# microsoft/ANCE

Measured on NVIDIA H100. Metric: ANN-refresh throughput: passages encoded/sec + queries top-200/sec, 8.8M x 768, higher is better.
Workload: dtype fp16

## Files before the change

### ance_b200/csrc/capi.cu

```cuda
#include <atomic>
#include <mutex>
#include <string.h>
#include <vector>

#include "common.h"
#include "gemm_store.cuh"

namespace ance {

static thread_local char g_err[1024] = "";
std::atomic<int64_t> g_launches{0};

void set_error(const char* fmt, ...) {
  va_list ap;
  va_start(ap, fmt);
  vsnprintf(g_err, sizeof(g_err), fmt, ap);
  va_end(ap);
}

void count_launch(int n) { g_launches.fetch_add(n, std::memory_order_relaxed); }

static bool g_prof_on = false;
static std::mutex g_prof_mu;
static std::vector<cudaEvent_t> g_ev_pool;
struct Span { cudaEvent_t a, b; };
static std::vector<Span> g_spans[kNumCls];
static cudaEvent_t g_open[kNumCls];
static double g_ms[kNumCls];
static int64_t g_cnt[kNumCls];

static cudaEvent_t get_event() {
  if (!g_ev_pool.empty()) { cudaEvent_t e = g_ev_pool.back(); g_ev_pool.pop_back(); return e; }
  cudaEvent_t e; cudaEventCreate(&e); return e;
}
void prof_begin(int cls, cudaStream_t st) {
  if (!g_prof_on) return;
  std::lock_guard<std::mutex> lk(g_prof_mu);
  g_open[cls] = get_event();
  cudaEventRecord(g_open[cls], st);
}
void prof_end(int cls, cudaStream_t st) {
  if (!g_prof_on) return;
  std::lock_guard<std::mutex> lk(g_prof_mu);
  cudaEvent_t b = get_event();
  cudaEventRecord(b, st);
  g_spans[cls].push_back({g_open[cls], b});
}

}

extern "C" const char* ance_version(void) { return "ance_b200 0.1 (sm_90a)"; }
extern "C" const char* ance_last_error(void) { return ance::g_err; }
extern "C" int64_t ance_launch_count(void) { return ance::g_launches.load(); }

extern "C" int ance_profile_enable(int on) {
  std::lock_guard<std::mutex> lk(ance::g_prof_mu);
  ance::g_prof_on = on != 0;
  return ANCE_OK;
}

extern "C" int ance_profile_read(double* ms_by_class, int64_t* launches_by_class, int n, int reset) {
  ANCE_REQUIRE(ms_by_class && launches_by_class && n > 0 && n <= ance::kNumCls, "ance_profile_read: bad arguments");
  ANCE_CUDA(cudaDeviceSynchronize());
  std::lock_guard<std::mutex> lk(ance::g_prof_mu);
  for (int c = 0; c < ance::kNumCls; ++c) {
    for (auto& s : ance::g_spans[c]) {
      float ms = 0.f;
      if (cudaEventElapsedTime(&ms, s.a, s.b) == cudaSuccess) { ance::g_ms[c] += ms; ance::g_cnt[c] += 1; }
      ance::g_ev_pool.push_back(s.a);
      ance::g_ev_pool.push_back(s.b);
    }
    ance::g_spans[c].clear();
  }
  for (int c = 0; c < n; ++c) { ms_by_class[c] = ance::g_ms[c]; launches_by_class[c] = ance::g_cnt[c]; }
  if (reset) for (int c = 0; c < ance::kNumCls; ++c) { ance::g_ms[c] = 0; ance::g_cnt[c] = 0; }
  return ANCE_OK;
}

namespace {

template <int BN, int STAGES, int CG, uint32_t FMT>
int run_dbg(const void* A, const void* B, int M, int N, int K, const float* bias, const void* R, int act, void* C,
            float* C32, cudaStream_t st) {
  constexpr int EW = 4;
  using Ep = gemm::EpStore<BN, EW>;
  CUtensorMap tmA, tmB;
  if (!tc05_host::make_tmap_2d_16b(&tmA, A, M, K, K, gemm::BM) ||
      !tc05_host::make_tmap_2d_16b(&tmB, B, N, K, K, BN / CG)) {
    ance::set_error("cuTensorMapEncodeTiled failed (M=%d N=%d K=%d)", M, N, K);
    return ANCE_ERR_CUDA;
  }
  gemm::WorkShape ws = gemm::make_shape(M, N, K, BN, CG, 0);
  typename Ep::Params p;
  memset(&p, 0, sizeof(p));
  if (C && !gemm::make_store_tmap(&p.tmC, C, M, N, N)) {
    ance::set_error("cuTensorMapEncodeTiled failed for the output (M=%d N=%d)", M, N);
    return ANCE_ERR_CUDA;
  }
  if (C && R && !gemm::make_store_tmap(&p.tmR, const_cast<void*>(R), M, N, N)) {
    ance::set_error("cuTensorMapEncodeTiled failed for the residual (M=%d N=%d)", M, N);
    return ANCE_ERR_CUDA;
  }
  p.C = reinterpret_cast<uint16_t*>(C);
  p.C32 = C32;
  p.bias = bias;
  p.R = reinterpret_cast<const uint16_t*>(R);
  p.ldc = N;
  p.ldc32 = N;
  p.ldr = N;
  p.act = act;
  ANCE_CUDA((gemm::launch<Ep, BN, STAGES, CG, EW, FMT>(tmA, tmB, ws, p, 0, st)));
  ance::count_launch(1);
  return ANCE_OK;
}

template <uint32_t FMT>
int dispatch_dbg(int variant, const void* A, const void* B, int M, int N, int K, const float* bias, const void* R,
                 int act, void* C, float* C32, cudaStream_t st) {
  switch (variant) {
    case 0: return run_dbg<128, 4, 1, FMT>(A, B, M, N, K, bias, R, act, C, C32, st);
    case 1: return run_dbg<128, 3, 1, FMT>(A, B, M, N, K, bias, R, act, C, C32, st);
    case 2: return run_dbg<128, 4, 2, FMT>(A, B, M, N, K, bias, R, act, C, C32, st);
    case 3: return run_dbg<64, 6, 2, FMT>(A, B, M, N, K, bias, R, act, C, C32, st);
    case 4: return run_dbg<64, 6, 1, FMT>(A, B, M, N, K, bias, R, act, C, C32, st);
    default: ance::set_error("ance_dbg_gemm: unknown variant %d", variant); return ANCE_ERR_INVALID;
  }
}

}

extern "C" int ance_dbg_gemm(const void* A_dev, const void* B_dev, int M, int N, int K, int fmt, int variant,
                             const float* bias_dev, const void* residual_bf16_dev, int act, void* C_bf16_dev,
                             float* C_f32_dev, void* stream) {
  ANCE_REQUIRE(A_dev && B_dev && M > 0 && N > 0 && K > 0, "ance_dbg_gemm: null operand or empty shape");
  ANCE_REQUIRE(K % 8 == 0 && N % 8 == 0, "ance_dbg_gemm: K and N must be multiples of 8 (16-byte rows)");
  cudaStream_t st = reinterpret_cast<cudaStream_t>(stream);
  if (fmt == ANCE_FMT_BF16)
    return dispatch_dbg<tc05::kFmtBF16>(variant, A_dev, B_dev, M, N, K, bias_dev, residual_bf16_dev, act, C_bf16_dev,
                                        C_f32_dev, st);
  if (fmt == ANCE_FMT_FP16)
    return dispatch_dbg<tc05::kFmtF16>(variant, A_dev, B_dev, M, N, K, bias_dev, residual_bf16_dev, act, C_bf16_dev,
                                       C_f32_dev, st);
  ance::set_error("ance_dbg_gemm: unknown operand format %d", fmt);
  return ANCE_ERR_INVALID;
}
```

### ance_b200/csrc/encoder.cu

```cuda
#include <math.h>
#include <stdlib.h>
#include <string.h>

#include <map>
#include <vector>

#include "attention.cuh"
#include "common.h"
#include "gemm_store.cuh"

namespace {

constexpr float kLog2e = 1.4426950408889634f;

struct EmbedParams {
  const int32_t* ids;
  const int32_t* lens;
  const uint8_t* mask;
  int B, L, H;
  int roberta;
  int pad_id, vocab, max_pos;
  const float* word;
  const float* pos;
  const float* type;
  const float* gamma;
  const float* beta;
  float eps;
  uint16_t* X;
  float* kbias;
  int* err_flag;
  const int32_t* seq_row0;
};

template <int NV, uint32_t FMT>
__global__ void __launch_bounds__(256) embed_ln_kernel(const EmbedParams p) {
  using A16 = act16::Act<FMT>;
  __shared__ int s_pos[512];
  __shared__ int s_warp_cnt[8];
  const int b = blockIdx.x;
  const int warp = threadIdx.x >> 5, lane = threadIdx.x & 31;
  const int32_t* ids = p.ids + static_cast<size_t>(b) * p.L;
  for (int base = 0, carry = 0; base < p.L; base += 256) {
    const int t = base + threadIdx.x;
    const int flag = (t < p.L && ids[t] != p.pad_id) ? 1 : 0;
    const unsigned bal = __ballot_sync(0xffffffffu, flag);
    if (lane == 0) s_warp_cnt[warp] = __popc(bal);
    __syncthreads();
    int pre = carry;
    for (int w2 = 0; w2 < warp; ++w2) pre += s_warp_cnt[w2];
    const int incl = pre + __popc(bal & ((2u << lane) - 1u));
    if (t < p.L) s_pos[t] = p.roberta ? (flag ? incl + p.pad_id : p.pad_id) : t;
    int tot = 0;
    for (int w2 = 0; w2 < 8; ++w2) tot += s_warp_cnt[w2];
    carry += tot;
    __syncthreads();
  }
  const int len = p.lens ? p.lens[b] : 0;
  const bool varlen = p.seq_row0 != nullptr;
  const size_t row0 = varlen ? static_cast<size_t>(p.seq_row0[b]) : static_cast<size_t>(b) * p.L;
  const int t_end = varlen ? min(len, p.L) : p.L;
  for (int t = warp; t < t_end; t += 8) {
    const size_t tok = row0 + t;
    int id = ids[t];
    int ps = s_pos[t];
    if (id < 0 || id >= p.vocab || ps >= p.max_pos) {
      if (lane == 0) atomicOr(p.err_flag, 1);
      id = min(max(id, 0), p.vocab - 1);
      ps = min(ps, p.max_pos - 1);
    }
    const float4* wr = reinterpret_cast<const float4*>(p.word + static_cast<size_t>(id) * p.H);
    const float4* pr = reinterpret_cast<const float4*>(p.pos + static_cast<size_t>(ps) * p.H);
    const float4* tr = reinterpret_cast<const float4*>(p.type);
    float x[NV * 8];
    float sum = 0.f;
#pragma unroll
    for (int v = 0; v < NV; ++v) {
#pragma unroll
      for (int hf = 0; hf < 2; ++hf) {
        const int c4 = (v * 32 + lane) * 2 + hf;
        const float4 a = __ldg(wr + c4), c = __ldg(pr + c4), d = __ldg(tr + c4);
        x[v * 8 + hf * 4 + 0] = (a.x + c.x) + d.x;
        x[v * 8 + hf * 4 + 1] = (a.y + c.y) + d.y;
        x[v * 8 + hf * 4 + 2] = (a.z + c.z) + d.z;
        x[v * 8 + hf * 4 + 3] = (a.w + c.w) + d.w;
      }
#pragma unroll
      for (int i = 0; i < 8; ++i) sum += x[v * 8 + i];
    }
#pragma unroll
    for (int s = 16; s > 0; s >>= 1) sum += __shfl_xor_sync(0xffffffffu, sum, s);
    const float mean = sum / p.H;
    float var = 0.f;
#pragma unroll
    for (int i = 0; i < NV * 8; ++i) {
      const float dlt = x[i] - mean;
      var = fmaf(dlt, dlt, var);
    }
#pragma unroll
    for (int s = 16; s > 0; s >>= 1) var += __shfl_xor_sync(0xffffffffu, var, s);
    const float rstd = rsqrtf(var / p.H + p.eps);
    uint4* out = reinterpret_cast<uint4*>(p.X + tok * p.H);
#pragma unroll
    for (int v = 0; v < NV; ++v) {
      const int col = (v * 32 + lane) * 8;
      const float4 g0 = __ldg(reinterpret_cast<const float4*>(p.gamma + col)), g1 = __ldg(reinterpret_cast<const float4*>(p.gamma + col + 4));
      const float4 b0 = __ldg(reinterpret_cast<const float4*>(p.beta + col)), b1 = __ldg(reinterpret_cast<const float4*>(p.beta + col + 4));
      const float g[8] = {g0.x, g0.y, g0.z, g0.w, g1.x, g1.y, g1.z, g1.w};
      const float bb[8] = {b0.x, b0.y, b0.z, b0.w, b1.x, b1.y, b1.z, b1.w};
      uint32_t h2[4];
#pragma unroll
      for (int q = 0; q < 4; ++q)
        h2[q] = A16::pack2((x[v * 8 + q * 2] - mean) * rstd * g[q * 2] + bb[q * 2],
                           (x[v * 8 + q * 2 + 1] - mean) * rstd * g[q * 2 + 1] + bb[q * 2 + 1]);
      out[v * 32 + lane] = make_uint4(h2[0], h2[1], h2[2], h2[3]);
    }
    if (lane == 0 && !varlen) {
      const bool keep = p.mask ? (p.mask[tok] != 0) : (t < len);
      p.kbias[tok] = keep ? 0.f : -10000.0f * kLog2e;
    }
  }
}

template <int NV, bool kInF32, uint32_t FMT>
__global__ void __launch_bounds__(256) ln_rows_kernel(const void* __restrict__ in, size_t in_ld, int n_rows, int H,
                                                      const float* __restrict__ gamma, const float* __restrict__ beta,
                                                      float eps, uint16_t* __restrict__ out16,
                                                      float* __restrict__ out32) {
  using A16 = act16::Act<FMT>;
  const int lane = threadIdx.x & 31;
  const int row = blockIdx.x * 8 + (threadIdx.x >> 5);
  if (row >= n_rows) return;
  float x[NV * 8];
  float sum = 0.f;
#pragma unroll
  for (int v = 0; v < NV; ++v) {
    const int col = (v * 32 + lane) * 8;
    if (kInF32) {
      const float* r = reinterpret_cast<const float*>(in) + static_cast<size_t>(row) * in_ld + col;
      const float4 a = __ldg(reinterpret_cast<const float4*>(r)), b = __ldg(reinterpret_cast<const float4*>(r + 4));
      x[v * 8 + 0] = a.x; x[v * 8 + 1] = a.y; x[v * 8 + 2] = a.z; x[v * 8 + 3] = a.w;
      x[v * 8 + 4] = b.x; x[v * 8 + 5] = b.y; x[v * 8 + 6] = b.z; x[v * 8 + 7] = b.w;
    } else {
      const uint16_t* r = reinterpret_cast<const uint16_t*>(in) + static_cast<size_t>(row) * in_ld + col;
      const uint4 a = __ldg(reinterpret_cast<const uint4*>(r));
      const uint32_t ah[4] = {a.x, a.y, a.z, a.w};
#pragma unroll
      for (int q = 0; q < 4; ++q) {
        const float2 f = A16::unpack2(ah[q]);
        x[v * 8 + q * 2] = f.x;
        x[v * 8 + q * 2 + 1] = f.y;
      }
    }
#pragma unroll
    for (int i = 0; i < 8; ++i) sum += x[v * 8 + i];
  }
#pragma unroll
  for (int s = 16; s > 0; s >>= 1) sum += __shfl_xor_sync(0xffffffffu, sum, s);
  const float mean = sum / H;
  float var = 0.f;
#pragma unroll
  for (int i = 0; i < NV * 8; ++i) {
    const float d = x[i] - mean;
// ... 110 lines not shown
  const int lane = threadIdx.x & 31;
  const int row0 = (blockIdx.x * 8 + (threadIdx.x >> 5)) * kB;
  if (row0 >= n_rows) return;
  uint4 raw[kB][NV];
  float sum[kB], var[kB], mean[kB], rstd[kB];
#pragma unroll
  for (int b = 0; b < kB; ++b) {
    const int row = min(row0 + b, n_rows - 1);
    const uint4* src = reinterpret_cast<const uint4*>(in + static_cast<size_t>(row) * in_ld);
#pragma unroll
    for (int v = 0; v < NV; ++v) raw[b][v] = __ldg(src + v * 32 + lane);
  }
#pragma unroll
  for (int b = 0; b < kB; ++b) {
    sum[b] = 0.f;
#pragma unroll
    for (int v = 0; v < NV; ++v) {
      const uint32_t w[4] = {raw[b][v].x, raw[b][v].y, raw[b][v].z, raw[b][v].w};
#pragma unroll
      for (int q = 0; q < 4; ++q) {
        const float2 f = A16::unpack2(w[q]);
        sum[b] += f.x;
        sum[b] += f.y;
      }
    }
  }
#pragma unroll
  for (int s = 16; s > 0; s >>= 1) {
#pragma unroll
    for (int b = 0; b < kB; ++b) sum[b] += __shfl_xor_sync(0xffffffffu, sum[b], s);
  }
#pragma unroll
  for (int b = 0; b < kB; ++b) {
    mean[b] = sum[b] / H;
    var[b] = 0.f;
#pragma unroll
    for (int v = 0; v < NV; ++v) {
      const uint32_t w[4] = {raw[b][v].x, raw[b][v].y, raw[b][v].z, raw[b][v].w};
#pragma unroll
      for (int q = 0; q < 4; ++q) {
        const float2 f = A16::unpack2(w[q]);
        const float d0 = f.x - mean[b], d1 = f.y - mean[b];
        var[b] = fmaf(d0, d0, var[b]);
        var[b] = fmaf(d1, d1, var[b]);
      }
    }
  }
#pragma unroll
  for (int s = 16; s > 0; s >>= 1) {
#pragma unroll
    for (int b = 0; b < kB; ++b) var[b] += __shfl_xor_sync(0xffffffffu, var[b], s);
  }
#pragma unroll
  for (int b = 0; b < kB; ++b) rstd[b] = rsqrtf(var[b] / H + eps);
#pragma unroll
  for (int v = 0; v < NV; ++v) {
    const int col = (v * 32 + lane) * 8;
    const float4 g0 = __ldg(reinterpret_cast<const float4*>(gamma + col)), g1 = __ldg(reinterpret_cast<const float4*>(gamma + col + 4));
    const float4 b0 = __ldg(reinterpret_cast<const float4*>(beta + col)), b1 = __ldg(reinterpret_cast<const float4*>(beta + col + 4));
    const float g[8] = {g0.x, g0.y, g0.z, g0.w, g1.x, g1.y, g1.z, g1.w};
    const float bb[8] = {b0.x, b0.y, b0.z, b0.w, b1.x, b1.y, b1.z, b1.w};
#pragma unroll
    for (int b = 0; b < kB; ++b) {
      const uint32_t w[4] = {raw[b][v].x, raw[b][v].y, raw[b][v].z, raw[b][v].w};
      uint32_t o[4];
#pragma unroll
      for (int q = 0; q < 4; ++q) {
        const float2 f = A16::unpack2(w[q]);
        o[q] = A16::pack2((f.x - mean[b]) * rstd[b] * g[q * 2] + bb[q * 2], (f.y - mean[b]) * rstd[b] * g[q * 2 + 1] + bb[q * 2 + 1]);
      }
      if (row0 + b < n_rows) *reinterpret_cast<uint4*>(out16 + static_cast<size_t>(row0 + b) * H + col) = make_uint4(o[0], o[1], o[2], o[3]);
    }
  }
}

__global__ void gather_rows16_by_index_kernel(const uint16_t* __restrict__ src, const int32_t* __restrict__ idx, int n, int H,
                                              uint16_t* __restrict__ dst) {
  const int r = blockIdx.x;
  if (r >= n) return;
  const uint4* s = reinterpret_cast<const uint4*>(src + static_cast<size_t>(idx[r]) * H);
  uint4* o = reinterpret_cast<uint4*>(dst + static_cast<size_t>(r) * H);
  for (int i = threadIdx.x; i < H / 8; i += blockDim.x) o[i] = __ldg(s + i);
}

template <uint32_t FMT>
__global__ void act16_to_f32_kernel(const uint16_t* __restrict__ in, float* __restrict__ out, size_t n) {
  const size_t i = static_cast<size_t>(blockIdx.x) * blockDim.x + threadIdx.x;
  if (i < n) out[i] = act16::Act<FMT>::to_float(in[i]);
}

__global__ void check_finite_kernel(const float* __restrict__ x, size_t n, int* __restrict__ err_flag) {
  bool bad = false;
  for (size_t i = static_cast<size_t>(blockIdx.x) * blockDim.x + threadIdx.x; i < n; i += static_cast<size_t>(gridDim.x) * blockDim.x)
    bad |= !(fabsf(x[i]) <= 3.0e38f);
  if (__any_sync(0xffffffffu, bad) && (threadIdx.x & 31) == 0) atomicOr(err_flag, 2);
}

}

struct LayerDev {
  uint16_t *wqkv, *wo, *w1, *w2;
  float *bqkv, *bo, *b1, *b2, *ln1g, *ln1b, *ln2g, *ln2b;
};

struct ance_encoder {
  ance_encoder_config cfg{};
  int max_tokens = 0;
  uint32_t fmt = tc05::kFmtF16;
  int device = 0;
  float *word = nullptr, *pos = nullptr, *type = nullptr;
  float *eg = nullptr, *eb = nullptr;
  std::vector<LayerDev> layers;
  uint16_t* head_w = nullptr;
  float *head_b = nullptr, *head_g = nullptr, *head_bt = nullptr;
  uint16_t *X = nullptr, *QKV = nullptr, *CTX = nullptr, *T = nullptr, *X1 = nullptr, *FF = nullptr;
  float* kbias = nullptr;
  uint16_t *cls_ctx = nullptr, *cls_x = nullptr;
  int32_t* seq_row0 = nullptr;
  uint8_t *row_lo = nullptr, *row_hi = nullptr;
  float* head_tmp = nullptr;
  int* err_flag = nullptr;
  uint16_t* dbg = nullptr;
  int dbg_tokens = 0;
  int prune_last_layer = 1;
  int varlen_align = 1;
  std::vector<void*> allocs;
};

namespace {

template <class T>
T* dev_alloc(ance_encoder* e, size_t n) {
  void* p = nullptr;
  if (cudaMalloc(&p, n * sizeof(T)) != cudaSuccess) return nullptr;
  e->allocs.push_back(p);
  return reinterpret_cast<T*>(p);
}

float* upload_f32(ance_encoder* e, const float* h, size_t n) {
  float* d = dev_alloc<float>(e, n);
  if (d) cudaMemcpy(d, h, n * 4, cudaMemcpyHostToDevice);
  return d;
}

uint16_t* upload_16(ance_encoder* e, const float* h, size_t n) {
  std::vector<uint16_t> tmp(n);
  if (e->fmt == tc05::kFmtBF16) for (size_t i = 0; i < n; ++i) tmp[i] = act16::Act<tc05::kFmtBF16>::from_float_host(h[i]);
  else for (size_t i = 0; i < n; ++i) tmp[i] = act16::Act<tc05::kFmtF16>::from_float_host(h[i]);
  uint16_t* d = dev_alloc<uint16_t>(e, n);
  if (d) cudaMemcpy(d, tmp.data(), n * 2, cudaMemcpyHostToDevice);
  return d;
}

template <uint32_t FMT>
int linear(const uint16_t* A, size_t lda, int M, const uint16_t* W, int N, int K, const float* bias,
           const uint16_t* R, int act, uint16_t* C, float* C32, cudaStream_t st, int cls = ance::kClsGemm,
           size_t ldr = 0) {
  constexpr int BN = 128, CG = 1, EW = 4, STAGES = 4;
  using Ep = gemm::EpStore<BN, EW, FMT>;
  CUtensorMap tmA, tmB;
  if (!tc05_host::make_tmap_2d_16b(&tmA, A, M, K, lda, gemm::BM) || !tc05_host::make_tmap_2d_16b(&tmB, W, N, K, K, BN / CG)) {
    ance::set_error("encoder: cuTensorMapEncodeTiled failed (M=%d N=%d K=%d)", M, N, K);
    return ANCE_ERR_CUDA;
  }
  gemm::WorkShape ws = gemm::make_shape(M, N, K, BN, CG, 0);
  typename Ep::Params p;
  memset(&p, 0, sizeof(p));
  if (C && !gemm::make_store_tmap(&p.tmC, C, M, N, N)) {
    ance::set_error("encoder: cuTensorMapEncodeTiled failed for the output (M=%d N=%d)", M, N);
    return ANCE_ERR_CUDA;
  }
  if (ldr == 0) ldr = N;
  if (C && R && !gemm::make_store_tmap(&p.tmR, const_cast<uint16_t*>(R), M, N, static_cast<int>(ldr))) {
    ance::set_error("encoder: cuTensorMapEncodeTiled failed for the residual (M=%d N=%d)", M, N);
    return ANCE_ERR_CUDA;
  }
  p.C = C;
  p.C32 = C32;
  p.bias = bias;
  p.R = R;
  p.ldc = N;
  p.ldc32 = N;
  p.ldr = static_cast<int>(ldr);
  static const int gelu_form = getenv("ANCE_B200_GELU") ? atoi(getenv("ANCE_B200_GELU")) : 2;
  p.act = act ? gelu_form : 0;
  {
    ance::ProfScope ps(cls, st);
    ANCE_CUDA((gemm::launch<Ep, BN, STAGES, CG, EW, FMT>(tmA, tmB, ws, p, 0, st)));
  }
  ance::count_launch(1);
  return ANCE_OK;
}

int g_ln_rows_per_warp = 2;

template <uint32_t FMT>
int layer_norm(const void* in, bool in_f32, size_t in_ld, int rows, int H, const float* g, const float* b, float eps,
               uint16_t* out16, float* out32, cudaStream_t st) {
  const int blocks = (rows + 7) / 8;
  const int nv = H / 256;
  ance::ProfScope ps(ance::kClsNorm, st);
  if (!in_f32 && out16 && !out32 && nv == 3 && g_ln_rows_per_warp > 1 && rows >= 4096) {
    const uint16_t* src = reinterpret_cast<const uint16_t*>(in);
    if (g_ln_rows_per_warp == 2) ln_rows_multi_kernel<3, 2, FMT><<<(rows + 15) / 16, 256, 0, st>>>(src, in_ld, rows, H, g, b, eps, out16);
    else if (g_ln_rows_per_warp == 3) ln_rows_packed_kernel<3, 2, FMT><<<(rows + 15) / 16, 256, 0, st>>>(src, in_ld, rows, H, g, b, eps, out16);
    else ln_rows_multi_kernel<3, 4, FMT><<<(rows + 31) / 32, 256, 0, st>>>(src, in_ld, rows, H, g, b, eps, out16);
    ANCE_CUDA(cudaGetLastError());
    ance::count_launch(1);
    return ANCE_OK;
  }
#define LN_CASE(NV_)                                                                                            \
  if (in_f32) ln_rows_kernel<NV_, true, FMT><<<blocks, 256, 0, st>>>(in, in_ld, rows, H, g, b, eps, out16, out32); \
  else ln_rows_kernel<NV_, false, FMT><<<blocks, 256, 0, st>>>(in, in_ld, rows, H, g, b, eps, out16, out32)
  if (nv == 3) { LN_CASE(3); }
  else if (nv == 4) { LN_CASE(4); }
  else if (nv == 1) { LN_CASE(1); }
  else if (nv == 2) { LN_CASE(2); }
  else { ance::set_error("encoder: hidden size %d unsupported", H); return ANCE_ERR_UNSUPPORTED; }
#undef LN_CASE
  ANCE_CUDA(cudaGetLastError());
  ance::count_launch(1);
  return ANCE_OK;
}

template <uint32_t FMT>
int set_attention_attrs() {
  ANCE_CUDA(cudaFuncSetAttribute(attn::attention_kernel<false, false, FMT>, cudaFuncAttributeMaxDynamicSharedMemorySize, attn::Smem::kDynamic));
  ANCE_CUDA(cudaFuncSetAttribute(attn::attention_kernel<false, true, FMT>, cudaFuncAttributeMaxDynamicSharedMemorySize, attn::Smem::kDynamic));
  ANCE_CUDA(cudaFuncSetAttribute(attn::attention_kernel<true, true, FMT>, cudaFuncAttributeMaxDynamicSharedMemorySize, attn::Smem::kDynamic));
  return ANCE_OK;
}

template <uint32_t FMT>
int forward_impl(ance_encoder* e, const int32_t* ids_dev, const int32_t* lens_dev, const uint8_t* mask_dev, int B, int L,
                 float* out_dev, cudaStream_t st, int n_tiles = 0) {
  const ance_encoder_config& c = e->cfg;
  const bool varlen = n_tiles > 0;
  const int M = varlen ? n_tiles * attn::kTile : B * L, H = c.hidden, F = c.ffn;
  int rc;
  if (varlen) {
    ANCE_CUDA(cudaMemsetAsync(e->X, 0, static_cast<size_t>(M) * H * 2, st));
    ANCE_CUDA(cudaMemsetAsync(e->kbias, 0, static_cast<size_t>(M) * 4, st));
  }
  EmbedParams ep;
  ep.ids = ids_dev; ep.lens = lens_dev; ep.mask = mask_dev;
  ep.B = B; ep.L = L; ep.H = H;
  ep.roberta = (c.arch == ANCE_ARCH_ROBERTA);
  ep.pad_id = c.pad_id; ep.vocab = c.vocab; ep.max_pos = c.max_pos;
  ep.word = e->word; ep.pos = e->pos; ep.type = e->type;
  ep.gamma = e->eg; ep.beta = e->eb; ep.eps = c.ln_eps;
  ep.X = e->X; ep.kbias = e->kbias; ep.err_flag = e->err_flag;
  ep.seq_row0 = varlen ? e->seq_row0 : nullptr;
  ance::prof_begin(ance::kClsNorm, st);
  switch (H / 256) {
    case 1: embed_ln_kernel<1, FMT><<<B, 256, 0, st>>>(ep); break;
    case 2: embed_ln_kernel<2, FMT><<<B, 256, 0, st>>>(ep); break;
    case 3: embed_ln_kernel<3, FMT><<<B, 256, 0, st>>>(ep); break;
    default: embed_ln_kernel<4, FMT><<<B, 256, 0, st>>>(ep); break;
  }
  ance::prof_end(ance::kClsNorm, st);
  ANCE_CUDA(cudaGetLastError());
  ance::count_launch(1);
  if (e->dbg && M <= e->dbg_tokens) ANCE_CUDA(cudaMemcpyAsync(e->dbg, e->X, static_cast<size_t>(M) * H * 2, cudaMemcpyDeviceToDevice, st));
  CUtensorMap tmQKV;
  if (!tc05_host::make_tmap_2d_16b(&tmQKV, e->QKV, M, 3 * H, 3 * H, attn::kTile)) {
    ance::set_error("encoder: cuTensorMapEncodeTiled failed for QKV");
    return ANCE_ERR_CUDA;
  }
  CUtensorMap tmCTX;
  if (!tc05_host::make_tmap_2d_16b(&tmCTX, e->CTX, M, H, H, attn::kTile)) {
    ance::set_error("encoder: cuTensorMapEncodeTiled failed for the attention output");
    return ANCE_ERR_CUDA;
  }
  attn::Params ap;
  ap.n_tokens = M; ap.L = varlen ? 64 : L; ap.heads = c.heads; ap.hidden = H;
  ap.kbias = e->kbias;
  ap.scale_log2 = kLog2e / 8.0f;
  ap.row_lo = varlen ? e->row_lo : nullptr;
  ap.row_hi = varlen ? e->row_hi : nullptr;
  const int attn_work = ((M + 127) / 128) * c.heads;
  const int attn_grid = std::min(attn_work, gemm::sm_count());
  for (int l = 0; l < c.n_layer; ++l) {
    const LayerDev& d = e->layers[l];
    if ((rc = linear<FMT>(e->X, H, M, d.wqkv, 3 * H, H, d.bqkv, nullptr, 0, e->QKV, nullptr, st, ance::kClsGemmQkv))) return rc;
    ance::prof_begin(ance::kClsAttn, st);
    if (varlen || L < attn::kTile) attn::attention_kernel<true, true, FMT><<<attn_grid, attn::kThreads, attn::Smem::kDynamic, st>>>(tmQKV, tmCTX, ap);
    else if (L == attn::kTile) attn::attention_kernel<false, true, FMT><<<attn_grid, attn::kThreads, attn::Smem::kDynamic, st>>>(tmQKV, tmCTX, ap);
    else attn::attention_kernel<false, false, FMT><<<attn_grid, attn::kThreads, attn::Smem::kDynamic, st>>>(tmQKV, tmCTX, ap);
    ance::prof_end(ance::kClsAttn, st);
    ANCE_CUDA(cudaGetLastError());
    ance::count_launch(1);
    const bool cls_only = (e->prune_last_layer || varlen) && (l == c.n_layer - 1);
    const int Mr = cls_only ? B : M;
    const uint16_t *ctx_a = e->CTX, *res_x = e->X;
    size_t pitch = cls_only ? static_cast<size_t>(L) * H : H;
    if (cls_only && varlen) {
      ance::ProfScope ps(ance::kClsNorm, st);
      gather_rows16_by_index_kernel<<<B, 96, 0, st>>>(e->CTX, e->seq_row0, B, H, e->cls_ctx);
      gather_rows16_by_index_kernel<<<B, 96, 0, st>>>(e->X, e->seq_row0, B, H, e->cls_x);
      ANCE_CUDA(cudaGetLastError());
      ance::count_launch(2);
      ctx_a = e->cls_ctx; res_x = e->cls_x; pitch = H;
    }
    if ((rc = linear<FMT>(ctx_a, pitch, Mr, d.wo, H, H, d.bo, res_x, 0, e->T, nullptr, st, ance::kClsGemmOut, pitch))) return rc;
    if ((rc = layer_norm<FMT>(e->T, false, H, Mr, H, d.ln1g, d.ln1b, c.ln_eps, e->X1, nullptr, st))) return rc;
    if ((rc = linear<FMT>(e->X1, H, Mr, d.w1, F, H, d.b1, nullptr, 1, e->FF, nullptr, st, ance::kClsGemmFfn1))) return rc;
    if ((rc = linear<FMT>(e->FF, F, Mr, d.w2, H, F, d.b2, e->X1, 0, e->T, nullptr, st, ance::kClsGemmFfn2))) return rc;
    if ((rc = layer_norm<FMT>(e->T, false, H, Mr, H, d.ln2g, d.ln2b, c.ln_eps, e->X, nullptr, st))) return rc;
    if (e->dbg && M <= e->dbg_tokens)
      ANCE_CUDA(cudaMemcpyAsync(e->dbg + static_cast<size_t>(l + 1) * e->dbg_tokens * H, e->X, static_cast<size_t>(Mr) * H * 2, cudaMemcpyDeviceToDevice, st));
  }
  const size_t cls_pitch = (e->prune_last_layer || varlen) ? static_cast<size_t>(H) : static_cast<size_t>(L) * H;
  if (c.has_head) {
    if ((rc = linear<FMT>(e->X, cls_pitch, B, e->head_w, H, H, e->head_b, nullptr, 0, nullptr, e->head_tmp, st))) return rc;
    if ((rc = layer_norm<FMT>(e->head_tmp, true, H, B, H, e->head_g, e->head_bt, 1e-5f, nullptr, out_dev, st))) return rc;
  } else {
    ance::ProfScope ps(ance::kClsNorm, st);
    gather_rows_f32_kernel<FMT><<<B, 256, 0, st>>>(e->X, cls_pitch, B, H, out_dev);
    ANCE_CUDA(cudaGetLastError());
    ance::count_launch(1);
  }
  {
    ance::ProfScope ps(ance::kClsNorm, st);
    const size_t n = static_cast<size_t>(B) * H;
    check_finite_kernel<<<static_cast<unsigned>(std::min<size_t>((n + 255) / 256, 148)), 256, 0, st>>>(out_dev, n, e->err_flag);
    ANCE_CUDA(cudaGetLastError());
    ance::count_launch(1);
  }
  return ANCE_OK;
}

}

extern "C" int ance_encoder_create(const ance_encoder_config* cfg, const ance_encoder_weights* w, int max_tokens,
                                   ance_encoder_t* out) {
  ANCE_REQUIRE(cfg && w && out, "ance_encoder_create: null argument");
  ANCE_REQUIRE(cfg->hidden % 256 == 0 && cfg->hidden <= 1024, "ance_encoder_create: hidden must be a multiple of 256 (<= 1024), got %d", cfg->hidden);
  ANCE_REQUIRE(cfg->heads * 64 == cfg->hidden, "ance_encoder_create: head_dim must be 64 (hidden %d, heads %d)", cfg->hidden, cfg->heads);
  ANCE_REQUIRE(cfg->ffn % 8 == 0 && cfg->n_layer > 0 && cfg->vocab > 0 && cfg->max_pos > 0, "ance_encoder_create: bad config");
  ANCE_REQUIRE(max_tokens >= 128, "ance_encoder_create: max_tokens must be >= 128");
  ANCE_REQUIRE(!cfg->has_head || (w->head_w && w->head_b && w->head_ln_g && w->head_ln_b), "ance_encoder_create: has_head without head weights");
// ... 261 lines not shown
```

### ance_b200/csrc/tc05.cuh

```cuda
#pragma once

#include <cuda.h>
#include <cuda_bf16.h>
#include <cuda_fp16.h>
#include <cuda_runtime.h>
#include <stdint.h>
#include <stdio.h>

namespace tc05 {

__device__ __forceinline__ uint32_t smem_u32(const void* p) {
  return static_cast<uint32_t>(__cvta_generic_to_shared(p));
}

__device__ __forceinline__ uint32_t cluster_ctarank() {
  uint32_t r;
  asm volatile("mov.u32 %0, %%cluster_ctarank;" : "=r"(r));
  return r;
}

__device__ __forceinline__ void cluster_sync_all() {
  asm volatile("barrier.cluster.arrive.release.aligned;\n" ::: "memory");
  asm volatile("barrier.cluster.wait.acquire.aligned;\n" ::: "memory");
}

constexpr uint64_t kEvictNormal = 0x1000000000000000ull;
constexpr uint64_t kEvictFirst  = 0x12F0000000000000ull;
constexpr uint64_t kEvictLast   = 0x14F0000000000000ull;

__device__ __forceinline__ void mbar_init(uint64_t* bar, uint32_t count) {
  asm volatile("mbarrier.init.shared::cta.b64 [%0], %1;" ::"r"(smem_u32(bar)), "r"(count) : "memory");
}

__device__ __forceinline__ void fence_barrier_init() {
  asm volatile("fence.mbarrier_init.release.cluster;" ::: "memory");
}

__device__ __forceinline__ void fence_proxy_async_smem() {
  asm volatile("fence.proxy.async.shared::cta;" ::: "memory");
}

__device__ __forceinline__ void mbar_arrive_expect_tx(uint64_t* bar, uint32_t bytes) {
  asm volatile("mbarrier.arrive.expect_tx.shared::cta.b64 _, [%0], %1;" ::"r"(smem_u32(bar)), "r"(bytes)
               : "memory");
}

__device__ __forceinline__ void mbar_arrive(uint64_t* bar) {
  asm volatile("mbarrier.arrive.shared::cta.b64 _, [%0];" ::"r"(smem_u32(bar)) : "memory");
}

__device__ __forceinline__ void mbar_arrive_cluster(uint64_t* bar, uint32_t cta) {
  uint32_t remote;
  asm volatile("mapa.shared::cluster.u32 %0, %1, %2;" : "=r"(remote) : "r"(smem_u32(bar)), "r"(cta));
  asm volatile("mbarrier.arrive.release.cluster.shared::cluster.b64 _, [%0];" ::"r"(remote) : "memory");
}

__device__ __forceinline__ uint32_t mbar_try_wait(uint64_t* bar, uint32_t parity) {
  uint32_t ok;
  asm volatile(
      "{\n\t"
      ".reg .pred p;\n\t"
      "mbarrier.try_wait.parity.shared::cta.b64 p, [%1], %2;\n\t"
      "selp.u32 %0, 1, 0, p;\n\t"
      "}"
      : "=r"(ok)
      : "r"(smem_u32(bar)), "r"(parity)
      : "memory");
  return ok;
}

#ifndef TC05_WATCHDOG_CYCLES
#define TC05_WATCHDOG_CYCLES 8000000000ll
#endif
__device__ __forceinline__ void mbar_wait(uint64_t* bar, uint32_t parity, int tag = 0) {
  (void)tag;
  if (mbar_try_wait(bar, parity)) return;
  long long t0 = clock64();
  uint32_t spins = 0;
  while (!mbar_try_wait(bar, parity)) {
    if ((++spins & 0x3FFu) == 0 && clock64() - t0 > TC05_WATCHDOG_CYCLES) asm volatile("trap;");
  }
}

__device__ __forceinline__ void tma_prefetch_desc(const CUtensorMap* tm) {
  asm volatile("prefetch.tensormap [%0];" ::"l"(reinterpret_cast<uint64_t>(tm)) : "memory");
}

__device__ __forceinline__ void tma_load_2d(void* smem_dst, const CUtensorMap* tm, uint64_t* bar, int c0,
                                            int c1, uint64_t hint) {
  asm volatile(
      "cp.async.bulk.tensor.2d.shared::cluster.global.mbarrier::complete_tx::bytes.L2::cache_hint"
      " [%0], [%1, {%3, %4}], [%2], %5;"
      :
      : "r"(smem_u32(smem_dst)), "l"(reinterpret_cast<uint64_t>(tm)), "r"(smem_u32(bar)), "r"(c0), "r"(c1),
        "l"(hint)
      : "memory");
}

__device__ __forceinline__ void tma_load_2d_multicast(void* smem_dst, const CUtensorMap* tm, uint64_t* bar, int c0,
                                                      int c1, uint16_t cta_mask, uint64_t hint) {
  asm volatile(
      "cp.async.bulk.tensor.2d.shared::cluster.global.mbarrier::complete_tx::bytes.multicast::cluster.L2::cache_hint"
      " [%0], [%1, {%3, %4}], [%2], %5, %6;"
      :
      : "r"(smem_u32(smem_dst)), "l"(reinterpret_cast<uint64_t>(tm)), "r"(smem_u32(bar)), "r"(c0), "r"(c1),
        "h"(cta_mask), "l"(hint)
      : "memory");
}

__device__ __forceinline__ void tma_store_2d(const CUtensorMap* tm, const void* smem_src, int c0, int c1) {
  asm volatile("cp.async.bulk.tensor.2d.global.shared::cta.bulk_group [%0, {%2, %3}], [%1];"
               :
               : "l"(reinterpret_cast<uint64_t>(tm)), "r"(smem_u32(smem_src)), "r"(c0), "r"(c1)
               : "memory");
}
__device__ __forceinline__ void bulk_commit_group() { asm volatile("cp.async.bulk.commit_group;" ::: "memory"); }
__device__ __forceinline__ void bulk_wait_read_all() { asm volatile("cp.async.bulk.wait_group.read 0;" ::: "memory"); }
__device__ __forceinline__ void bulk_wait_all() { asm volatile("cp.async.bulk.wait_group 0;" ::: "memory"); }

__device__ __forceinline__ void named_bar_sync(int id, int threads) {
  asm volatile("bar.sync %0, %1;" ::"r"(id), "r"(threads) : "memory");
}

__device__ __forceinline__ uint64_t make_desc_k_sw128(uint32_t smem_addr) {
  uint64_t d = 0;
  d |= static_cast<uint64_t>((smem_addr & 0x3FFFFu) >> 4);
  d |= static_cast<uint64_t>(1) << 16;
  d |= static_cast<uint64_t>(1024 >> 4) << 32;
  d |= static_cast<uint64_t>(1) << 62;
  return d;
}

__device__ __forceinline__ uint64_t make_desc_mn_sw128(uint32_t smem_addr, uint32_t lbo_bytes,
                                                       uint32_t sbo_bytes) {
  uint64_t d = 0;
  d |= static_cast<uint64_t>((smem_addr & 0x3FFFFu) >> 4);
  d |= static_cast<uint64_t>((lbo_bytes >> 4) & 0x3FFFu) << 16;
  d |= static_cast<uint64_t>((sbo_bytes >> 4) & 0x3FFFu) << 32;
  d |= static_cast<uint64_t>(1) << 62;
  return d;
}

enum : uint32_t { kFmtF16 = 0, kFmtBF16 = 1 };

__device__ __forceinline__ void wgmma_fence() { asm volatile("wgmma.fence.sync.aligned;" ::: "memory"); }
__device__ __forceinline__ void wgmma_commit() { asm volatile("wgmma.commit_group.sync.aligned;" ::: "memory"); }
template <int N>
__device__ __forceinline__ void wgmma_wait() { asm volatile("wgmma.wait_group.sync.aligned %0;" ::"n"(N) : "memory"); }
template <int R>
__device__ __forceinline__ void wgmma_fence_regs(float (&d)[R]) {
#pragma unroll
  for (int i = 0; i < R; ++i) asm volatile("" : "+f"(d[i])::"memory");
}

#define TC05_R8(i) "+f"(d[i]), "+f"(d[i + 1]), "+f"(d[i + 2]), "+f"(d[i + 3]), "+f"(d[i + 4]), "+f"(d[i + 5]), "+f"(d[i + 6]), "+f"(d[i + 7])
#define TC05_R32 TC05_R8(0), TC05_R8(8), TC05_R8(16), TC05_R8(24)
#define TC05_R64 TC05_R32, TC05_R8(32), TC05_R8(40), TC05_R8(48), TC05_R8(56)
#define TC05_S32                                                                  \
  "%0, %1, %2, %3, %4, %5, %6, %7, %8, %9, %10, %11, %12, %13, %14, %15, "        \
  "%16, %17, %18, %19, %20, %21, %22, %23, %24, %25, %26, %27, %28, %29, %30, %31"
#define TC05_S64                                                                  \
  TC05_S32 ", "                                                                   \
  "%32, %33, %34, %35, %36, %37, %38, %39, %40, %41, %42, %43, %44, %45, %46, %47, " \
  "%48, %49, %50, %51, %52, %53, %54, %55, %56, %57, %58, %59, %60, %61, %62, %63"
#define TC05_WGMMA(NAME, INSTR, NR, SLIST, RLIST, IA, IB, IP, IT)                                                     \
  template <int kTransB>                                                                                              \
  __device__ __forceinline__ void NAME(float (&d)[NR], uint64_t adesc, uint64_t bdesc, uint32_t accumulate) {        \
    asm volatile("{\n\t.reg .pred p;\n\tsetp.ne.b32 p, %" IP ", 0;\n\t" INSTR " {" SLIST "}, %" IA ", %" IB           \
                 ", p, 1, 1, 0, %" IT ";\n\t}"                                                                        \
                 : RLIST                                                                                              \
                 : "l"(adesc), "l"(bdesc), "r"(accumulate), "n"(kTransB));                                            \
  }
TC05_WGMMA(wgmma_m64n128k16_bf16, "wgmma.mma_async.sync.aligned.m64n128k16.f32.bf16.bf16", 64, TC05_S64, TC05_R64, "64", "65", "66", "67")
TC05_WGMMA(wgmma_m64n128k16_f16, "wgmma.mma_async.sync.aligned.m64n128k16.f32.f16.f16", 64, TC05_S64, TC05_R64, "64", "65", "66", "67")
TC05_WGMMA(wgmma_m64n64k16_bf16, "wgmma.mma_async.sync.aligned.m64n64k16.f32.bf16.bf16", 32, TC05_S32, TC05_R32, "32", "33", "34", "35")
TC05_WGMMA(wgmma_m64n64k16_f16, "wgmma.mma_async.sync.aligned.m64n64k16.f32.f16.f16", 32, TC05_S32, TC05_R32, "32", "33", "34", "35")

template <uint32_t FMT, int kTransB>
__device__ __forceinline__ void wgmma_n128(float (&d)[64], uint64_t adesc, uint64_t bdesc, uint32_t accumulate) {
  if constexpr (FMT == kFmtBF16) wgmma_m64n128k16_bf16<kTransB>(d, adesc, bdesc, accumulate);
  else wgmma_m64n128k16_f16<kTransB>(d, adesc, bdesc, accumulate);
}
template <uint32_t FMT, int kTransB>
__device__ __forceinline__ void wgmma_n64(float (&d)[32], uint64_t adesc, uint64_t bdesc, uint32_t accumulate) {
  if constexpr (FMT == kFmtBF16) wgmma_m64n64k16_bf16<kTransB>(d, adesc, bdesc, accumulate);
  else wgmma_m64n64k16_f16<kTransB>(d, adesc, bdesc, accumulate);
}

template <int R>
__device__ __forceinline__ void acc_store_frag(float* tile, int pitch, int r0, int c0, const float (&d)[R]) {
  const int t = threadIdx.x & 127;
  const int r = r0 + 16 * (t >> 5) + ((t & 31) >> 2);
  const int c = c0 + 2 * (t & 3);
#pragma unroll
  for (int j = 0; j < R / 4; ++j) {
    *reinterpret_cast<float2*>(tile + r * pitch + c + 8 * j) = make_float2(d[4 * j], d[4 * j + 1]);
    *reinterpret_cast<float2*>(tile + (r + 8) * pitch + c + 8 * j) = make_float2(d[4 * j + 2], d[4 * j + 3]);
  }
}

__device__ __forceinline__ void acc_ld_x32(uint32_t waddr, uint32_t* v) {
#pragma unroll
  for (int i = 0; i < 32; i += 4)
    asm volatile("ld.shared.v4.u32 {%0, %1, %2, %3}, [%4];"
                 : "=r"(v[i]), "=r"(v[i + 1]), "=r"(v[i + 2]), "=r"(v[i + 3])
                 : "r"((waddr + i) * 4u)
                 : "memory");
}

template <int kStages>
struct Ring {
  uint32_t stage = 0, phase = 0;
  __device__ __forceinline__ void advance() {
    if (++stage == kStages) {
      stage = 0;
      phase ^= 1;
    }
  }
};

}

namespace tc05_host {

typedef CUresult (*EncodeTiledFn)(CUtensorMap*, CUtensorMapDataType, cuuint32_t, void*, const cuuint64_t*,
                                  const cuuint64_t*, const cuuint32_t*, const cuuint32_t*, CUtensorMapInterleave,
                                  CUtensorMapSwizzle, CUtensorMapL2promotion, CUtensorMapFloatOOBfill);

inline EncodeTiledFn encode_fn() {
  static EncodeTiledFn fn = nullptr;
  if (!fn) {
    void* p = nullptr;
    cudaDriverEntryPointQueryResult q;
    if (cudaGetDriverEntryPoint("cuTensorMapEncodeTiled", &p, cudaEnableDefault, &q) != cudaSuccess ||
        q != cudaDriverEntryPointSuccess)
      return nullptr;
    fn = reinterpret_cast<EncodeTiledFn>(p);
  }
  return fn;
}

inline bool make_tmap_2d_16b(CUtensorMap* tm, const void* base, uint64_t rows, uint64_t cols, uint64_t ld_elems,
                             uint32_t box_rows, uint32_t box_cols = 64) {
  EncodeTiledFn fn = encode_fn();
  if (!fn) return false;
  cuuint64_t gdim[2] = {cols, rows};
  cuuint64_t gstride[1] = {ld_elems * 2};
  cuuint32_t box[2] = {box_cols, box_rows};
  cuuint32_t estr[2] = {1, 1};
  CUresult r = fn(tm, CU_TENSOR_MAP_DATA_TYPE_BFLOAT16, 2, const_cast<void*>(base), gdim, gstride, box, estr,
                  CU_TENSOR_MAP_INTERLEAVE_NONE, CU_TENSOR_MAP_SWIZZLE_128B, CU_TENSOR_MAP_L2_PROMOTION_L2_256B,
                  CU_TENSOR_MAP_FLOAT_OOB_FILL_NONE);
  return r == CUDA_SUCCESS;
}

}
```

Before: 13300.

## Add warp-specialized persistent wgmma GEMM for large-K linear layers

Adds a persistent, warp-specialized GEMM kernel. One producer warpgroup issues TMA loads into a 5-stage ring, and two consumer warpgroups alternate output tiles with setmaxnreg register rebalancing and ping-pong ordering barriers. The epilogue (bias, GELU, residual via TMA) is fused and results go out through TMA stores. The encoder routes linear layers with K>=2048 (the FFN down-projection, K=3072) to this kernel, so epilogue and mainloop work can overlap across tiles. This adds complexity and a higher smem footprint, and the residual path loads residual tiles into the same output buffers, which needs careful synchronization.

```diff
diff --git a/ance_b200/csrc/capi.cu b/ance_b200/csrc/capi.cu
--- a/ance_b200/csrc/capi.cu
+++ b/ance_b200/csrc/capi.cu
@@ -4,7 +4,7 @@
 #include <vector>
 
 #include "common.h"
-#include "gemm_store.cuh"
+#include "gemm_ws.cuh"
 
 namespace ance {
 
@@ -123,6 +123,16 @@
     case 2: return run_dbg<128, 4, 2, FMT>(A, B, M, N, K, bias, R, act, C, C32, st);
     case 3: return run_dbg<64, 6, 2, FMT>(A, B, M, N, K, bias, R, act, C, C32, st);
     case 4: return run_dbg<64, 6, 1, FMT>(A, B, M, N, K, bias, R, act, C, C32, st);
+    case 5: {
+      const cudaError_t e = gemm::ws::linear<FMT, tc05::kFmtBF16>(A, K, M, B, N, K, bias, R, N, act, C, C32, st);
+      if (e == cudaErrorInvalidPitchValue) {
+        ance::set_error("cuTensorMapEncodeTiled failed (M=%d N=%d K=%d)", M, N, K);
+        return ANCE_ERR_CUDA;
+      }
+      ANCE_CUDA(e);
+      ance::count_launch(1);
+      return ANCE_OK;
+    }
     default: ance::set_error("ance_dbg_gemm: unknown variant %d", variant); return ANCE_ERR_INVALID;
   }
 }
diff --git a/ance_b200/csrc/encoder.cu b/ance_b200/csrc/encoder.cu
--- a/ance_b200/csrc/encoder.cu
+++ b/ance_b200/csrc/encoder.cu
@@ -7,7 +7,7 @@
 
 #include "attention.cuh"
 #include "common.h"
-#include "gemm_store.cuh"
+#include "gemm_ws.cuh"
 
 namespace {
 
@@ -424,6 +424,7 @@
   return d;
 }
 
+constexpr int kWsMinK = 2048;
 template <uint32_t FMT>
 int linear(const uint16_t* A, size_t lda, int M, const uint16_t* W, int N, int K, const float* bias,
            const uint16_t* R, int act, uint16_t* C, float* C32, cudaStream_t st, int cls = ance::kClsGemm,
@@ -458,7 +459,11 @@
   p.act = act ? gelu_form : 0;
   {
     ance::ProfScope ps(cls, st);
-    ANCE_CUDA((gemm::launch<Ep, BN, STAGES, CG, EW, FMT>(tmA, tmB, ws, p, 0, st)));
+    if (K >= kWsMinK) {
+      ANCE_CUDA((gemm::ws::linear<FMT, FMT>(A, lda, M, W, N, K, bias, R, ldr, p.act, C, C32, st)));
+    } else {
+      ANCE_CUDA((gemm::launch<Ep, BN, STAGES, CG, EW, FMT>(tmA, tmB, ws, p, 0, st)));
+    }
   }
   ance::count_launch(1);
   return ANCE_OK;
diff --git a/ance_b200/csrc/gemm_ws.cuh b/ance_b200/csrc/gemm_ws.cuh
--- /dev/null
+++ b/ance_b200/csrc/gemm_ws.cuh
@@ -0,0 +1,258 @@
+#pragma once
+#include "gemm_store.cuh"
+
+namespace gemm {
+namespace ws {
+
+constexpr int BN = 128;
+constexpr int STAGES = 5;
+constexpr int kThreads = 384;
+constexpr int kSubBytes = BM * 128;
+
+struct Plan {
+  static constexpr int kABytes = BM * BK * 2;
+  static constexpr int kBBytes = BN * BK * 2;
+  static constexpr int kStageBytes = kABytes + kBBytes;
+  static constexpr int kOutOffset = STAGES * kStageBytes;
+  static constexpr int kOutBytes = 2 * 2 * kSubBytes;
+  static constexpr int kBarOffset = kOutOffset + kOutBytes;
+  static constexpr int kBarBytes = (2 * STAGES + 6) * 8;
+  static constexpr int kDynamicBytes = kBarOffset + kBarBytes + 1024;
+  static_assert(kDynamicBytes <= 232448, "GEMM shared memory exceeds 227 KB");
+};
+
+struct alignas(64) Params {
+  CUtensorMap tmC;
+  CUtensorMap tmR;
+  float* C32;
+  const float* bias;
+  int M, N, K;
+  int ldc32;
+  int act;
+  int has_c;
+};
+
+template <uint32_t FMT, uint32_t OUT_FMT, bool RES>
+__global__ void __launch_bounds__(kThreads, 1)
+ws_gemm_kernel(const __grid_constant__ CUtensorMap tmA, const __grid_constant__ CUtensorMap tmB,
+               const __grid_constant__ Params p) {
+  using A16 = act16::Act<OUT_FMT>;
+
+  extern __shared__ uint8_t smem_raw[];
+  uint8_t* smem = reinterpret_cast<uint8_t*>((reinterpret_cast<uintptr_t>(smem_raw) + 1023) & ~uintptr_t(1023));
+  uint8_t* out_smem = smem + Plan::kOutOffset;
+  uint64_t* full_bar = reinterpret_cast<uint64_t*>(smem + Plan::kBarOffset);
+  uint64_t* empty_bar = full_bar + STAGES;
+  uint64_t* order_bar = empty_bar + STAGES;
+  uint64_t* rfull_bar = order_bar + 2;
+  uint64_t* rempty_bar = rfull_bar + 2;
+
+  const int wg = threadIdx.x >> 7;
+  const int num_n_blks = (p.N + BN - 1) / BN;
+  const int total = ((p.M + BM - 1) / BM) * num_n_blks;
+  const int num_kb = (p.K + BK - 1) / BK;
+
+  if (threadIdx.x == 0) {
+    tma_prefetch_desc(&tmA);
+    tma_prefetch_desc(&tmB);
+    for (int s = 0; s < STAGES; ++s) {
+      mbar_init(&full_bar[s], 1);
+      mbar_init(&empty_bar[s], 4);
+    }
+    for (int g = 0; g < 2; ++g) {
+      mbar_init(&order_bar[g], 1);
+      mbar_init(&rfull_bar[g], 1);
+      mbar_init(&rempty_bar[g], 1);
+    }
+    fence_barrier_init();
+  }
+  __syncthreads();
+
+  if (wg == 0) {
+    setmaxnreg_dec<40>();
+    if (threadIdx.x == 0) {
+      Ring<STAGES> ring;
+      uint32_t rphases = 0;
+      int i = 0;
+      for (int t = blockIdx.x; t < total; t += gridDim.x, ++i) {
+        const int m0 = (t / num_n_blks) * BM, n0 = (t % num_n_blks) * BN;
+        for (int kb = 0; kb < num_kb; ++kb) {
+          mbar_wait(&empty_bar[ring.stage], ring.phase ^ 1, 1);
+          uint8_t* sa = smem + ring.stage * Plan::kStageBytes;
+          mbar_arrive_expect_tx(&full_bar[ring.stage], Plan::kStageBytes);
+          tma_load_2d(sa, &tmA, &full_bar[ring.stage], kb * BK, m0, kEvictNormal);
+          tma_load_2d(sa + Plan::kABytes, &tmB, &full_bar[ring.stage], kb * BK, n0, kEvictLast);
+          ring.advance();
+          if constexpr (RES) {
+            if (kb == min(STAGES, num_kb) - 1) {
+              const int g = i & 1;
+              mbar_wait(&rempty_bar[g], ((rphases >> g) & 1) ^ 1, 5);
+              const int nsub = min(2, (p.N - n0 + 63) / 64);
+              mbar_arrive_expect_tx(&rfull_bar[g], nsub * kSubBytes);
+              for (int s = 0; s < nsub; ++s)
+                tma_load_2d(out_smem + (2 * g + s) * kSubBytes, &p.tmR, &rfull_bar[g], n0 + 64 * s, m0, kEvictFirst);
+              rphases ^= 1u << g;
+            }
+          }
+        }
+      }
+    }
+  } else {
+    setmaxnreg_inc<232>();
+    const int g = wg - 1;
+    const int lane = threadIdx.x & 31;
+    const int r = 16 * ((threadIdx.x >> 5) & 3) + (lane >> 2);
+    const int cq = 2 * (lane & 3);
+    const bool issuer = (threadIdx.x & 127) == 0;
+    const uint32_t off_r = r * 128 + 4 * (lane & 3);
+    uint32_t ord_phase = 0, rphase = 0, out_seq = 0;
+    auto release = [&](int stage) {
+      __syncwarp();
+      if (lane == 0) mbar_arrive(&empty_bar[stage]);
+    };
+    int i = g;
+    for (int t = blockIdx.x + g * gridDim.x; t < total; t += 2 * gridDim.x, i += 2) {
+      const int m0 = (t / num_n_blks) * BM, n0 = (t % num_n_blks) * BN;
+      if (i > 0) {
+        mbar_wait(&order_bar[g], ord_phase, 7);
+        ord_phase ^= 1;
+      }
+      float acc[2][64];
+#pragma unroll
+      for (int k = 0; k < 64; ++k) acc[0][k] = acc[1][k] = 0.f;
+      uint32_t pos = static_cast<uint32_t>(i) * num_kb;
+      int prev_stage = -1;
+      for (int kb = 0; kb < num_kb; ++kb, ++pos) {
+        const int stage = pos % STAGES;
+        mbar_wait(&full_bar[stage], (pos / STAGES) & 1, 3);
+        if (kb == num_kb - 1 && issuer) mbar_arrive(&order_bar[g ^ 1]);
+        const uint32_t sa = smem_u32(smem + stage * Plan::kStageBytes);
+        const uint32_t sb = sa + Plan::kABytes;
+        wgmma_fence();
+#pragma unroll
+        for (int k = 0; k < BK / MMA_K; ++k) {
+          const uint64_t bdesc = make_desc_k_sw128(sb + k * MMA_K * 2);
+          wgmma_n128<FMT, 0>(acc[0], make_desc_k_sw128(sa + k * MMA_K * 2), bdesc, 1u);
+          wgmma_n128<FMT, 0>(acc[1], make_desc_k_sw128(sa + 64 * 128 + k * MMA_K * 2), bdesc, 1u);
+        }
+        wgmma_commit();
+        wgmma_wait<1>();
+        wgmma_fence_regs(acc[0]);
+        wgmma_fence_regs(acc[1]);
+        if (prev_stage >= 0) release(prev_stage);
+        prev_stage = stage;
+      }
+      wgmma_wait<0>();
+      wgmma_fence_regs(acc[0]);
+      wgmma_fence_regs(acc[1]);
+      if (prev_stage >= 0) release(prev_stage);
+
+      if constexpr (RES) {
+        mbar_wait(&rfull_bar[g], rphase, 6);
+        rphase ^= 1;
+      }
+#pragma unroll
+      for (int s = 0; s < 2; ++s) {
+        const int col_s = n0 + 64 * s;
+        if (col_s < p.N) {
+          uint8_t* buf = out_smem + (2 * g + (RES ? s : (out_seq & 1))) * kSubBytes;
+          if (!RES && p.has_c) {
+            if (issuer) bulk_wait_read<1>();
+            named_bar_sync(1 + g, 128);
+          }
+#pragma unroll
+          for (int h = 0; h < 2; ++h) {
+            const int row_a = m0 + 64 * h + r, row_b = row_a + 8;
+#pragma unroll
+            for (int jj = 0; jj < 8; ++jj) {
+              const int j = 8 * s + jj;
+              const int col = col_s + 8 * jj + cq;
+              float v0 = acc[h][4 * j], v1 = acc[h][4 * j + 1], v2 = acc[h][4 * j + 2], v3 = acc[h][4 * j + 3];
+              if (p.bias && col < p.N) {
+                const float2 b = __ldg(reinterpret_cast<const float2*>(p.bias + col));
+                v0 += b.x; v1 += b.y; v2 += b.x; v3 += b.y;
+              }
+              if (p.act == 1) {
+                gelu_erf2(v0, v1);
+                gelu_erf2(v2, v3);
+              } else if (p.act == 2) {
+                gelu_logistic2(v0, v1);
+                gelu_logistic2(v2, v3);
+              }
+              uint32_t* pa = reinterpret_cast<uint32_t*>(buf + h * 64 * 128 + off_r + ((jj ^ (r & 7)) << 4));
+              uint32_t* pb = pa + 8 * 128 / 4;
+              if constexpr (RES) {
+                const float2 xa = A16::unpack2(*pa), xb = A16::unpack2(*pb);
+                v0 += xa.x; v1 += xa.y; v2 += xb.x; v3 += xb.y;
+              }
+              if (p.C32 && col < p.N) {
+                if (row_a < p.M) *reinterpret_cast<float2*>(p.C32 + (size_t)row_a * p.ldc32 + col) = make_float2(v0, v1);
+                if (row_b < p.M) *reinterpret_cast<float2*>(p.C32 + (size_t)row_b * p.ldc32 + col) = make_float2(v2, v3);
+              }
+              if (p.has_c) {
+                *pa = A16::pack2(v0, v1);
+                *pb = A16::pack2(v2, v3);
+              }
+            }
+          }
+          if (p.has_c) {
+            fence_proxy_async_smem();
+            named_bar_sync(1 + g, 128);
+            if (issuer) {
+              tma_store_2d(&p.tmC, buf, col_s, m0);
+              bulk_commit_group();
+            }
+            ++out_seq;
+          } else if (RES) {
+            named_bar_sync(1 + g, 128);
+          }
+        }
+      }
+      if (RES && issuer) {
+        if (p.has_c) bulk_wait_read<0>();
+        mbar_arrive(&rempty_bar[g]);
+      }
+    }
+    if (issuer && p.has_c) bulk_wait_all();
+  }
+}
+
+template <uint32_t FMT, uint32_t OUT_FMT, bool RES>
+cudaError_t launch(const CUtensorMap& tmA, const CUtensorMap& tmB, const Params& p, cudaStream_t stream) {
+  auto kern = ws_gemm_kernel<FMT, OUT_FMT, RES>;
+  static bool configured[kMaxDevices] = {};
+  const int dev = current_device();
+  if (!configured[dev]) {
+    cudaError_t e = cudaFuncSetAttribute(kern, cudaFuncAttributeMaxDynamicSharedMemorySize, Plan::kDynamicBytes);
+    if (e != cudaSuccess) return e;
+    configured[dev] = true;
+  }
+  const int tiles = ((p.M + BM - 1) / BM) * ((p.N + BN - 1) / BN);
+  kern<<<min(tiles, sm_count()), kThreads, Plan::kDynamicBytes, stream>>>(tmA, tmB, p);
+  return cudaGetLastError();
+}
+
+template <uint32_t FMT, uint32_t OUT_FMT>
+cudaError_t linear(const void* A, size_t lda, int M, const void* W, int N, int K, const float* bias, const void* R,
+                   size_t ldr, int act, void* C, float* C32, cudaStream_t st) {
+  CUtensorMap tmA, tmB;
+  Params p;
+  memset(&p, 0, sizeof(p));
+  if (!tc05_host::make_tmap_2d_16b(&tmA, A, M, K, lda, BM) || !tc05_host::make_tmap_2d_16b(&tmB, W, N, K, K, BN) ||
+      (C && !tc05_host::make_tmap_2d_16b(&p.tmC, C, M, N, N, BM)) ||
+      (R && !tc05_host::make_tmap_2d_16b(&p.tmR, R, M, N, ldr, BM)))
+    return cudaErrorInvalidPitchValue;
+  p.C32 = C32;
+  p.bias = bias;
+  p.M = M;
+  p.N = N;
+  p.K = K;
+  p.ldc32 = N;
+  p.act = act;
+  p.has_c = C != nullptr;
+  if (R) return launch<FMT, OUT_FMT, true>(tmA, tmB, p, st);
+  return launch<FMT, OUT_FMT, false>(tmA, tmB, p, st);
+}
+
+}
+}
diff --git a/ance_b200/csrc/tc05.cuh b/ance_b200/csrc/tc05.cuh
--- a/ance_b200/csrc/tc05.cuh
+++ b/ance_b200/csrc/tc05.cuh
@@ -116,11 +116,18 @@
 }
 __device__ __forceinline__ void bulk_commit_group() { asm volatile("cp.async.bulk.commit_group;" ::: "memory"); }
 __device__ __forceinline__ void bulk_wait_read_all() { asm volatile("cp.async.bulk.wait_group.read 0;" ::: "memory"); }
+template <int N>
+__device__ __forceinline__ void bulk_wait_read() { asm volatile("cp.async.bulk.wait_group.read %0;" ::"n"(N) : "memory"); }
 __device__ __forceinline__ void bulk_wait_all() { asm volatile("cp.async.bulk.wait_group 0;" ::: "memory"); }
 
 __device__ __forceinline__ void named_bar_sync(int id, int threads) {
   asm volatile("bar.sync %0, %1;" ::"r"(id), "r"(threads) : "memory");
 }
+
+template <int N>
+__device__ __forceinline__ void setmaxnreg_dec() { asm volatile("setmaxnreg.dec.sync.aligned.u32 %0;" ::"n"(N)); }
+template <int N>
+__device__ __forceinline__ void setmaxnreg_inc() { asm volatile("setmaxnreg.inc.sync.aligned.u32 %0;" ::"n"(N)); }
 
 __device__ __forceinline__ uint64_t make_desc_k_sw128(uint32_t smem_addr) {
   uint64_t d = 0;
```

Result: no change. 13370 (median of 6 runs) (+0.5%).
